# CrystalAnalyst/Lsm

Hardware: AMD Instinct MI355X
Metric: GiB/s device-resident SSTable block encode+decode, 4 KiB blocks, 1/2/4/8 GPU (higher is better)
Workload: dtype u8; 1 GPU; U: 1048576 blocks/GPU x block_size 4096, decode + re-encode (16-B uniform keys, 100-B values); blocks_per_gpu=1048576, entries_per_gpu=32474205, encoded_bytes_per_gpu=4226189427, decoded_bytes_per_gpu=4286595060, block_size=4096, segments_per_gpu=2045, parallelism=block-sharded x1 (no data-path collective), encode_output=segments packed (lsmblk_encode_batch), rccl_world=1

## Files before the change

### lsm_amd/csrc/lsmblk_dev.hpp

```cpp
#pragma once

#include <hip/hip_runtime.h>
#include <hip/hip_ext.h>

#include <cstdint>
#include <cstdlib>
#include <cstring>
#include <mutex>
#include <new>
#include <type_traits>
#include <vector>

#include "lsmblk.h"

namespace {

typedef unsigned int u32x4 __attribute__((ext_vector_type(4)));
typedef unsigned int u32x2 __attribute__((ext_vector_type(2)));
typedef __amdgpu_buffer_rsrc_t rsrc_t;

constexpr uint32_t kSpinLimit = 1u << 22;

constexpr bool kDiag = LSMBLK_DIAG_BUILD != 0;
__device__ __forceinline__ uint32_t diag_mask(uint32_t skip) { return kDiag ? skip : 0u; }

__device__ __forceinline__ uint32_t lane_id() { return threadIdx.x & 63u; }
__device__ __forceinline__ uint32_t uni(uint32_t x) { return __builtin_amdgcn_readfirstlane(x); }

__device__ __forceinline__ uint32_t xcd_tile(uint32_t b, uint32_t G) {
  const uint32_t x = b & 7, i = b >> 3, q = G >> 3, r = G & 7;
  return x * q + (x < r ? x : r) + i;
}
__device__ __forceinline__ uint64_t uni64(uint64_t x) {
  return (uint64_t(uni(uint32_t(x >> 32))) << 32) | uni(uint32_t(x));
}
__device__ __forceinline__ uint64_t lane64(uint64_t x, uint32_t j) {
  return (uint64_t(uint32_t(__builtin_amdgcn_readlane(uint32_t(x >> 32), j))) << 32) |
         uint32_t(__builtin_amdgcn_readlane(uint32_t(x), j));
}
typedef const __attribute__((address_space(4))) uint32_t cu32_t;
typedef const __attribute__((address_space(4))) uint64_t cu64_t;
__device__ __forceinline__ cu32_t* kconst(const uint32_t* p) { return (cu32_t*)p; }
__device__ __forceinline__ cu64_t* kconst(const uint64_t* p) { return (cu64_t*)p; }
__device__ __forceinline__ uint32_t wave_id() { return __builtin_amdgcn_readfirstlane(threadIdx.x >> 6); }
__device__ __forceinline__ void wave_sync() {
  __builtin_amdgcn_fence(__ATOMIC_RELEASE, "wavefront");
  __builtin_amdgcn_wave_barrier();
  __builtin_amdgcn_fence(__ATOMIC_ACQUIRE, "wavefront");
}
#define LSM_DPP(v, ctrl, rmask) uint32_t(__builtin_amdgcn_update_dpp(0u, (v), (ctrl), (rmask), 0xF, false))
__device__ __forceinline__ uint32_t wave_incl_scan32(uint32_t v) {
  v += LSM_DPP(v, 0x111, 0xF);
  v += LSM_DPP(v, 0x112, 0xF);
  v += LSM_DPP(v, 0x114, 0xF);
  v += LSM_DPP(v, 0x118, 0xF);
  v += LSM_DPP(v, 0x142, 0xA);
  v += LSM_DPP(v, 0x143, 0xC);
  return v;
}
__device__ __forceinline__ uint32_t wave_incl_max32(uint32_t v) {
  v = max(v, LSM_DPP(v, 0x111, 0xF));
  v = max(v, LSM_DPP(v, 0x112, 0xF));
  v = max(v, LSM_DPP(v, 0x114, 0xF));
  v = max(v, LSM_DPP(v, 0x118, 0xF));
  v = max(v, LSM_DPP(v, 0x142, 0xA));
  v = max(v, LSM_DPP(v, 0x143, 0xC));
  return v;
}
__device__ __forceinline__ uint32_t wave_incl_min31(uint32_t v) { return 0x7FFFFFFFu - wave_incl_max32(0x7FFFFFFFu - v); }
__device__ __forceinline__ uint32_t wave_sum32(uint32_t v) {
  return __builtin_amdgcn_readlane(wave_incl_scan32(v), 63);
}
template <typename T>
__device__ __forceinline__ T wave_incl_scan(T v) {
  if constexpr (sizeof(T) == 4) {
    return T(wave_incl_scan32(uint32_t(v)));
  } else {
    const uint32_t l = lane_id();
#pragma unroll
    for (uint32_t d = 1; d < 64; d <<= 1) {
      T t = __shfl_up(v, d, 64);
      if (l >= d) v += t;
    }
    return v;
  }
}
template <typename T>
__device__ __forceinline__ T wave_sum(T v) {
  if constexpr (sizeof(T) == 4) {
    return T(__builtin_amdgcn_readlane(wave_incl_scan32(uint32_t(v)), 63));
  } else {
#pragma unroll
    for (uint32_t d = 32; d >= 1; d >>= 1) v += __shfl_xor(v, d, 64);
    return v;
  }
}
__device__ __forceinline__ rsrc_t make_rsrc(const void* p16, uint32_t nbytes) {
  const uint32_t n = nbytes >= 0xFFFFFFF0u ? 0xFFFFFFFFu : (nbytes + 15) & ~15u;
  return __builtin_amdgcn_make_buffer_rsrc(const_cast<void*>(p16), (short)0, (int)n, 0x00020000);
}
__device__ __forceinline__ rsrc_t make_rsrc_exact(void* p16, uint32_t nbytes) {
  return __builtin_amdgcn_make_buffer_rsrc(p16, (short)0, (int)nbytes, 0x00020000);
}
__device__ __forceinline__ uint32_t bswap16(uint32_t v) { return ((v & 0xFF) << 8) | ((v >> 8) & 0xFF); }

__device__ __forceinline__ uint64_t gload(const uint64_t* p, uint32_t poll) {
  if (poll == 2)
    return __hip_atomic_fetch_or(const_cast<uint64_t*>(p), 0ull, __ATOMIC_RELAXED, __HIP_MEMORY_SCOPE_AGENT);
  return __hip_atomic_load(p, __ATOMIC_RELAXED, __HIP_MEMORY_SCOPE_AGENT);
}
__device__ __forceinline__ void gstore(uint64_t* p, uint64_t v, uint32_t poll) {
  if (poll == 2)
    (void)__hip_atomic_exchange(p, v, __ATOMIC_RELAXED, __HIP_MEMORY_SCOPE_AGENT);
  else
    __hip_atomic_store(p, v, __ATOMIC_RELAXED, __HIP_MEMORY_SCOPE_AGENT);
}

// ... 854 lines not shown
```

### lsm_amd/csrc/lsmblk_gpu.hip

```cpp
#include "lsmblk_dev.hpp"

namespace {


struct DecodeArgs {
  const uint8_t* blocks;
  const uint64_t* blk_off;
  uint64_t nblk;
  uint8_t* keys;
  uint32_t* key_off;
  uint8_t* vals;
  uint32_t* val_off;
  uint64_t* ts;
  uint64_t entry_cap, key_cap, val_cap;
  uint64_t* stats;
  const uint32_t* agg;
  const uint64_t* tile_pre;
  uint32_t tail;
  uint64_t* blk_ent;
  uint32_t skip;
  uint64_t* bagg;
  uint64_t* bbase;
  uint64_t* tagg;
  uint64_t* tinc;
  uint64_t lag;
  uint64_t lag_bytes;
  uint64_t* dbg;
  uint32_t tag, poll;
};

constexpr uint32_t kTile = 64;
constexpr uint32_t kDbgTiles = 32768, kDbgWords = 16 + 8 * kDbgTiles;
__device__ __forceinline__ void dbg_trace(uint64_t* dbg, uint64_t t, uint32_t k) {
  if (kDiag && dbg && t < kDbgTiles && lane_id() == 0) dbg[16 + 8 * t + k] = __builtin_amdgcn_s_memrealtime();
}


constexpr uint32_t kLB = 2;
constexpr uint32_t kDecMB = 2;
#ifndef LSMBLK_XEB
#define LSMBLK_XEB 4
#endif
constexpr uint32_t kEB = LSMBLK_XEB;
constexpr uint32_t kEBBlock = 2;


constexpr uint32_t kDecImg = 4128;
constexpr uint32_t kDecMaxE = 128;
constexpr uint32_t kDecKeyImg = 2176;
constexpr uint32_t kDecMapN = 256;
constexpr uint32_t kDecOut = 4032;
static_assert(kDecOut <= 16 * kDecMapN && 16 * kDecMapN <= kDecImg, "the chunk map covers the value run");

struct alignas(16) DecLds {
  uint8_t img[kDecImg];
  alignas(16) uint8_t kimg[kDecKeyImg];
  alignas(16) uint16_t cmap[kDecMapN];
};
static_assert(sizeof(DecLds) <= (160 << 10) / 24, "decode LDS: room for 24 blocks per CU");

struct DecTables {
  uint16_t epos[kDecMaxE], pfx[kDecMaxE], sfx[kDecMaxE];
  uint32_t kout[kDecMaxE + 1], vout[kDecMaxE + 1];
};
static_assert(sizeof(DecTables) <= kDecImg, "large-block tables overlay the image");

struct DecEnt {
  uint32_t epos, p, s, kout, vout, vl;
};

__device__ __forceinline__ void lds_read16(const uint8_t* base, uint32_t x, uint32_t (&v)[4]) {
  const u32x4 q = *reinterpret_cast<const u32x4*>(base + x);
  v[0] = q.x, v[1] = q.y, v[2] = q.z, v[3] = q.w;
}

constexpr int kLdAux = 0;

template <class Img>
__device__ void dec_simple_outputs(const DecodeArgs& a, const Img& im, const BlockHdr& h,
                                   uint64_t E0, uint64_t K0, uint64_t V0) {
  const uint32_t l = lane_id();
  uint64_t kc = 0, vc = 0;
  for (uint32_t c = 0; c < h.n; c += 64) {
    const uint32_t k = c + l;
    uint32_t off = 0, p = 0, s = 0, vl = 0;
    if (k < h.n) parse_entry(im, h, k, off, p, s, vl);
    const uint64_t kl = p + s;
    const uint64_t ki = wave_incl_scan<uint64_t>(kl), vi = wave_incl_scan<uint64_t>(vl);
    const uint64_t kpos = K0 + kc + ki - kl, vpos = V0 + vc + vi - vl;
    kc += __shfl(ki, 63, 64);
    vc += __shfl(vi, 63, 64);
    if (k < h.n) {
      const uint64_t e = E0 + k;
      if (e < a.entry_cap) {
        a.ts[e] = im.u64(off + 4 + s);
        a.key_off[e] = uint32_t(kpos);
        a.val_off[e] = uint32_t(vpos);
      }
      for (uint32_t t = 0; t < p; ++t)
        if (kpos + t < a.key_cap) a.keys[kpos + t] = uint8_t(im.u8(4 + t));
      for (uint32_t t = 0; t < s; ++t)
        if (kpos + p + t < a.key_cap) a.keys[kpos + p + t] = uint8_t(im.u8(off + 4 + t));
      for (uint32_t t = 0; t < vl; ++t)
        if (vpos + t < a.val_cap) a.vals[vpos + t] = uint8_t(im.u8(off + 14 + s + t));
    }
  }
}

__device__ __forceinline__ void st16(const rsrc_t& R, uint32_t off, const uint32_t (&v)[4]) {
  const u32x4 q = {v[0], v[1], v[2], v[3]};
  __builtin_amdgcn_raw_buffer_store_b128(q, R, off, 0, 0);
}

__device__ __forceinline__ void st_short(const rsrc_t& R, uint32_t off, uint32_t len, const uint32_t (&v)[4]) {
// ... 412 lines not shown
  if (total == 0) {
    after(first, 0u, ~0u);
    return;
  }
  wave_sync();
  reinterpret_cast<u32x4*>(sc)[l] = u32x4{so, dof, len - 16, first};
  uint32_t carry = 0;
  for (uint32_t g0 = 0; g0 < total; g0 += 64 * B) {
    CopyBatch<B> c;
    copy_issue<B, PIN>(RS, g0, total, np, first, sc, carry, c);
    if constexpr (PIN) copy_land(c);
    copy_store(RD, c);
    after(first, g0, g0 + 64 * B >= total ? ~0u : g0 + 64 * B);
  }
}

__device__ __forceinline__ void dec_big_entry(const DecodeArgs& a, const DecTables& L, const GlbImg& im, uint32_t k,
                                              uint32_t lim, const rsrc_t& RK, uint32_t kb, uint64_t E0, uint64_t K0,
                                              uint64_t V0) {
  const rsrc_t& R = im.r;
  const uint32_t lead = im.lead, fk = lead + 4;
  const uint32_t epos = L.epos[k], p = L.pfx[k], s = L.sfx[k], kout = L.kout[k];
  const uint32_t sb = lead + epos + 4, kl = p + s;
  const uint64_t e = E0 + k;
  a.ts[e] = im.u64(epos + 4 + s);
  a.key_off[e] = uint32_t(K0 + kout);
  a.val_off[e] = uint32_t(V0 + L.vout[k]);
  for (uint32_t t = 0; t < kl; t += 16) {
    const uint32_t o = kl >= 16 ? min(t, kl - 16) : 0u;
    uint32_t v[4];
    if (sb + o >= p && sb + o - p + 16 <= lim && fk + o + 16 <= lim) {
      const u32x4 sq = gload16(R, sb + o - p), fq = gload16(R, fk + o);
      const uint32_t sv[4] = {sq.x, sq.y, sq.z, sq.w}, fv[4] = {fq.x, fq.y, fq.z, fq.w};
#pragma unroll
      for (uint32_t d = 0; d < 4; ++d) {
        const int32_t nf = int32_t(p) - int32_t(o + 4 * d);
        const uint32_t m = nf <= 0 ? 0u : nf >= 4 ? ~0u : (1u << (8 * nf)) - 1;
        v[d] = (fv[d] & m) | (sv[d] & ~m);
      }
    } else {
#pragma unroll
      for (uint32_t d = 0; d < 4; ++d) {
        uint32_t wd = 0;
        for (uint32_t i = 0; i < 4; ++i) {
          const uint32_t x = o + 4 * d + i;
          wd |= (x < p ? im.u8(4 + x) : im.u8(epos + 4 + x - p)) << (8 * i);
        }
        v[d] = wd;
      }
    }
    if (kl >= 16) st16(RK, kb + kout + o, v);
    else st_short(RK, kb + kout, kl, v);
  }
}

#ifndef LSMBLK_XDBB
#define LSMBLK_XDBB 8
#endif
constexpr uint32_t kDecBigB = LSMBLK_XDBB;

__device__ void dec_big_outputs(const DecodeArgs& a, const DecTables& L, const rsrc_t& R, uint32_t lead,
                                const BlockHdr& h, uint32_t n, uint64_t Eb, uint64_t K0, uint64_t V0, uint32_t K,
                                uint32_t V, uint32_t* sc) {
  const uint32_t l = lane_id();
  const uint32_t kb = uint32_t(K0 & 15), vb = uint32_t(V0 & 15);
  const rsrc_t RK = make_rsrc_exact(a.keys + (K0 - kb), kb + K), RV = make_rsrc_exact(a.vals + (V0 - vb), vb + V);
  const GlbImg im{R, lead};
  const uint32_t lim = lead + h.len;
  for (uint32_t c = 0; c < n; c += 64) {
    const uint32_t k = c + l;
    const bool live = k < n;
    uint32_t vsrc = 0, vdst = 0, vl = 0;
    if (live) {
      dec_big_entry(a, L, im, k, lim, RK, kb, Eb, K0, V0);
      vsrc = lead + L.epos[k] + 14 + L.sfx[k];
      vdst = vb + L.vout[k];
      vl = L.vout[k + 1] - L.vout[k];
      if (vl < kCoop) copy_run(R, vsrc, lim, RV, vdst, vl);
    }
    copy_long_runs<kDecBigB, true>(live && vl >= kCoop, R, vsrc, RV, vdst, vl, sc);
  }
}

template <bool lagm, class Mid, class Post, class PreWait>
__device__ void decode_block(const DecodeArgs& a, DecLds& L, uint64_t b, uint64_t start, uint64_t end, Mid&& mid,
                             Post&& post, PreWait&& pre_wait) {
  const uint32_t l = lane_id();
  uint32_t err = 0;
  const uint64_t tb = b / kTile, jb = b % kTile;
  uint32_t cn = 0, ck = 0, cv = 0;
  uint64_t tp0 = 0, tp1 = 0, tp2 = 0, gb = 0;
  if constexpr (!lagm) {
    if (l < jb) {
      const uint64_t q = tb * kTile + l;
      cn = a.agg[3 * q];
      ck = a.agg[3 * q + 1];
      cv = a.agg[3 * q + 2];
    }
    tp0 = a.tile_pre[3 * tb], tp1 = a.tile_pre[3 * tb + 1], tp2 = a.tile_pre[3 * tb + 2];
  }
  uint32_t len = 0;
  if (end < start + a.tail || end - start > 0x7FFFFFF0ull) err |= LSMBLK_ERR_MALFORMED;
  else len = uint32_t(end - start) - a.tail;
  const uint8_t* bp = a.blocks + start;
  const uint32_t lead = uni(uint32_t(reinterpret_cast<uintptr_t>(bp) & 15));
  const uint8_t* abase = bp - lead;
  const rsrc_t R = make_rsrc(abase, lead + len);
  const bool fits = lead + len + 15 <= kDecImg;

  BlockHdr h;
  if (fits) {
    const uint32_t nchunk = (lead + len + 15) >> 4;
    u32x4 v[5];
    if constexpr (lagm) {
      const uint32_t o = 16 * l, o4 = o + 4096;
      asm volatile(
          "s_nop 4\n\t"
          "buffer_load_dwordx4 %0, %5, %7, 0 offen\n\t"
          "buffer_load_dwordx4 %1, %5, %7, 0 offen offset:1024\n\t"
          "buffer_load_dwordx4 %2, %5, %7, 0 offen offset:2048\n\t"
          "buffer_load_dwordx4 %3, %5, %7, 0 offen offset:3072\n\t"
          "buffer_load_dwordx4 %4, %6, %7, 0 offen"
          : "=&v"(v[0]), "=&v"(v[1]), "=&v"(v[2]), "=&v"(v[3]), "=&v"(v[4])
          : "v"(o), "v"(o4), "s"(R));
      mid();
      asm volatile("s_waitcnt vmcnt(0)" ::: "memory");
#pragma unroll
      for (uint32_t i = 0; i < 5; ++i) asm volatile("" : "+v"(v[i]));
    } else {
#pragma unroll
      for (uint32_t i = 0; i < 5; ++i)
        v[i] = __builtin_amdgcn_raw_buffer_load_b128(R, (l + 64 * i) * 16, 0, kLdAux);
    }
#pragma unroll
    for (uint32_t i = 0; i < 5; ++i)
      if (l + 64 * i < nchunk) *reinterpret_cast<u32x4*>(L.img + (l + 64 * i) * 16) = v[i];
    wave_sync();
    post();
    if (lagm && l < 3 && !(diag_mask(a.skip) & 4096)) gb = gload(a.bbase + 3 * b + l, 0);
    h = parse_hdr(LdsImg{L.img, lead}, len);
  } else {
    mid();
    post();
    if (lagm && l < 3 && !(diag_mask(a.skip) & 4096)) gb = gload(a.bbase + 3 * b + l, 0);
    h = parse_hdr(GlbImg{R, lead}, len);
  }
  if (diag_mask(a.skip) & 256) return;
  if (!h.ok) err |= LSMBLK_ERR_MALFORMED;
  const bool fast = fits && h.n <= kDecMaxE;
  const bool big = !fits;

  uint64_t K = 0, V = 0;
  bool bad = false;
  DecTables& T = *reinterpret_cast<DecTables*>(L.img);
  auto parse_tables = [&](const auto& im, uint32_t c0, uint32_t cn, uint64_t& kr, uint64_t& vr) {
    for (uint32_t c = 0; c < cn; c += 64) {
      const uint32_t k = c + l;
      uint32_t off = 0, p = 0, s = 0, vl = 0;
      bool ok = true;
      if (k < cn) ok = parse_entry(im, h, c0 + k, off, p, s, vl);
      bad = bad || !ok;
      const uint32_t kl = p + s;
      const uint32_t ki = wave_incl_scan<uint32_t>(kl), vi = wave_incl_scan<uint32_t>(vl);
      if (k < cn) {
        T.epos[k] = uint16_t(off);
        T.pfx[k] = uint16_t(p);
        T.sfx[k] = uint16_t(s);
        T.kout[k] = uint32_t(kr) + ki - kl;
        T.vout[k] = uint32_t(vr) + vi - vl;
      }
      kr += __shfl(ki, 63, 64);
      vr += __shfl(vi, 63, 64);
    }
    if (l == 0) {
      T.kout[cn] = uint32_t(kr);
      T.vout[cn] = uint32_t(vr);
    }
  };
  DecEnt ent[2] = {};
  if (fast) {
    const LdsImg im{L.img, lead};
#pragma unroll
    for (uint32_t it = 0; it < 2; ++it) {
      if (64 * it >= h.n) break;
      const uint32_t k = 64 * it + l;
      uint32_t off = 0, p = 0, s = 0, vl = 0;
      bool ok = true;
      if (k < h.n) ok = parse_entry(im, h, k, off, p, s, vl);
      bad = bad || !ok;
      const uint32_t kl = p + s;
      const uint32_t ki = wave_incl_scan<uint32_t>(kl), vi = wave_incl_scan<uint32_t>(vl);
      ent[it] = DecEnt{off, p, s, uint32_t(K) + ki - kl, uint32_t(V) + vi - vl, vl};
      K += __shfl(ki, 63, 64);
      V += __shfl(vi, 63, 64);
    }
  } else if (big && h.n <= kDecMaxE) {
    parse_tables(GlbImg{R, lead}, 0, h.n, K, V);
  } else {
    for (uint32_t c = 0; c < h.n; c += 64) {
      const uint32_t k = c + l;
      uint32_t off = 0, p = 0, s = 0, vl = 0;
      bool ok = true;
      if (k < h.n) {
        if (fits) ok = parse_entry(LdsImg{L.img, lead}, h, k, off, p, s, vl);
        else ok = parse_entry(GlbImg{R, lead}, h, k, off, p, s, vl);
      }
      bad = bad || !ok;
      K += wave_sum<uint64_t>(p + s);
      V += wave_sum<uint64_t>(vl);
    }
  }
  if (diag_mask(a.skip) & 512) return;
  if (__ballot(bad)) err |= LSMBLK_ERR_MALFORMED;
  uint64_t agg[3] = {h.n, K, V};
  if (err) agg[0] = agg[1] = agg[2] = 0;

  pre_wait();
  uint64_t excl[3];
  if constexpr (lagm) {
    const uint64_t want = (uint64_t(a.tag) << 2) | 2;
    uint32_t spins = 0;
    if (b % kTile == 0) dbg_trace(a.dbg, b / kTile, 2);
    while (!(diag_mask(a.skip) & 2048) && __ballot(l < 3 && (gb & 0xFFFF) != want)) {
      if (++spins > kSpinLimit) {
        err |= LSMBLK_ERR_TIMEOUT;
        break;
      }
      __builtin_amdgcn_s_sleep(1);
      if (l < 3 && (gb & 0xFFFF) != want) gb = gload(a.bbase + 3 * b + l, a.poll);
    }
#pragma unroll
    for (uint32_t q = 0; q < 3; ++q)
      excl[q] = uint64_t(uint32_t(__builtin_amdgcn_readlane(uint32_t(gb >> 16), q))) |
                (uint64_t(uint32_t(__builtin_amdgcn_readlane(uint32_t(gb >> 48), q))) << 32);
    if (b % kTile == 0) dbg_trace(a.dbg, b / kTile, 3);
  } else {
    excl[0] = tp0 + wave_sum(cn);
    excl[1] = tp1 + wave_sum(ck);
    excl[2] = tp2 + wave_sum(cv);
  }
  wave_sync();
  const uint64_t E0 = excl[0], K0 = excl[1], V0 = excl[2];
  if (a.blk_ent && l == 0) a.blk_ent[b] = E0;
  const uint64_t Et = E0 + agg[0], Kt = K0 + agg[1], Vt = V0 + agg[2];
  if (Kt > 0xFFFFFFFFull || Vt > 0xFFFFFFFFull) err |= LSMBLK_ERR_OVERFLOW;
  if (Et > a.entry_cap || Kt > a.key_cap || Vt > a.val_cap) err |= LSMBLK_ERR_CAPACITY;
  if (lagm && b + 1 == a.nblk && l == 0) {
    if (a.blk_ent) a.blk_ent[a.nblk] = Et;
    a.stats[0] = Et;
    a.stats[1] = Kt;
    a.stats[2] = Vt;
    if (Et <= a.entry_cap) {
      a.key_off[Et] = uint32_t(Kt);
      a.val_off[Et] = uint32_t(Vt);
    }
  }

  if (!(err & (LSMBLK_ERR_MALFORMED | LSMBLK_ERR_TIMEOUT | LSMBLK_ERR_OVERFLOW | LSMBLK_ERR_CAPACITY)) && h.n) {
    if (fast) {
      dec_fast_outputs(a, L, lead, h, ent, E0, K0, V0, uint32_t(K), uint32_t(V), diag_mask(a.skip));
    } else if (big && h.n <= kDecMaxE) {
      dec_big_outputs(a, T, R, lead, h, h.n, E0, K0, V0, uint32_t(K), uint32_t(V), reinterpret_cast<uint32_t*>(L.kimg));
    } else if (big) {
      uint64_t kr = 0, vr = 0;
      for (uint32_t c0 = 0; c0 < h.n; c0 += kDecMaxE) {
        const uint32_t nc = min(kDecMaxE, h.n - c0);
        wave_sync();
        parse_tables(GlbImg{R, lead}, c0, nc, kr, vr);
        wave_sync();
        dec_big_outputs(a, T, R, lead, h, nc, E0 + c0, K0, V0, uint32_t(K), uint32_t(V), reinterpret_cast<uint32_t*>(L.kimg));
      }
    } else if (fits) {
      dec_simple_outputs(a, LdsImg{L.img, lead}, h, E0, K0, V0);
    } else {
      dec_simple_outputs(a, GlbImg{R, lead}, h, E0, K0, V0);
    }
  }
  raise_err(a.stats, err);
}

__global__ __launch_bounds__(64) __attribute__((amdgpu_waves_per_eu(5))) void decode_kernel(DecodeArgs a) {
  __shared__ DecLds lds;
  const uint64_t b = blockIdx.x;
  decode_block<false>(a, lds, b, uni64(a.blk_off[b]), uni64(a.blk_off[b + 1]), [] {}, [] {}, [] {});
}


__device__ __forceinline__ uint64_t sat47(uint64_t v) { return v > (1ull << 47) - 1 ? (1ull << 47) - 1 : v; }

__device__ __forceinline__ void publish3(uint64_t* arr, uint64_t idx, uint64_t x0, uint64_t x1, uint64_t x2,
                                         uint32_t tag, uint32_t flag, uint32_t poll) {
  const uint32_t l = lane_id();
  const uint64_t x = l == 0 ? x0 : (l == 1 ? x1 : x2);
  if (l < 3) gstore(arr + 3 * idx + l, (sat47(x) << 16) | (uint64_t(tag) << 2) | flag, poll);
}

struct BlkCount {
  uint32_t n;
  uint64_t K, V;
  bool bad;
};
struct CntPre {
  rsrc_t R;
  uint32_t len, lead;
  bool ok, staged;
  u32x4 v[5];
};
__device__ __forceinline__ CntPre cnt_issue(const uint8_t* blocks, uint32_t tail, uint64_t start, uint64_t end) {
  const uint32_t l = lane_id();
  CntPre C;
  C.ok = !(end < start + tail || end - start > 0x7FFFFFF0ull);
  C.len = C.ok ? uint32_t(end - start) - tail : 0u;
  const uint8_t* bp = blocks + start;
  C.lead = uni(uint32_t(reinterpret_cast<uintptr_t>(bp) & 15));
  C.R = make_rsrc(bp - C.lead, C.lead + C.len);
  C.staged = C.ok && C.lead + C.len + 15 <= kDecImg;
  if (C.staged) {
#pragma unroll
    for (uint32_t i = 0; i < 5; ++i)
      C.v[i] = __builtin_amdgcn_raw_buffer_load_b128(C.R, (l + 64 * i) * 16, 0, kLdAux);
  }
  return C;
}
__device__ __forceinline__ BlkCount cnt_finish(const CntPre& C, uint8_t* img) {
  const uint32_t l = lane_id();
  BlkCount r{0, 0, 0, false};
  bool bad = false;
  auto count = [&](const auto& im) {
    const BlockHdr h = parse_hdr(im, C.len);
    if (!h.ok) {
      bad = true;
      return;
    }
    r.n = h.n;
    if constexpr (std::is_same_v<std::decay_t<decltype(im)>, GlbImg>) {
      for (uint32_t c = 0; c < h.n; c += 128) {
        const uint32_t k0 = c + l, k1 = c + 64 + l;
        const bool l0 = k0 < h.n, l1 = k1 < h.n;
        uint32_t o0, p0, s0, v0, o1, p1, s1, v1;
        const bool ok0 = parse_entry(im, h, l0 ? k0 : h.n - 1, o0, p0, s0, v0);
        const bool ok1 = parse_entry(im, h, l1 ? k1 : h.n - 1, o1, p1, s1, v1);
        if ((l0 && !ok0) || (l1 && !ok1)) bad = true;
        r.K += wave_sum<uint32_t>((l0 ? p0 + s0 : 0u) + (l1 ? p1 + s1 : 0u));
        r.V += wave_sum<uint32_t>((l0 ? v0 : 0u) + (l1 ? v1 : 0u));
      }
    } else {
      for (uint32_t c = 0; c < h.n; c += 64) {
        const uint32_t k = c + l;
        uint32_t off = 0, p = 0, s = 0, vl = 0;
        if (k < h.n && !parse_entry(im, h, k, off, p, s, vl)) bad = true;
        r.K += wave_sum<uint32_t>(p + s);
        r.V += wave_sum<uint32_t>(vl);
      }
    }
  };
  if (C.staged) {
    const uint32_t nchunk = (C.lead + C.len + 15) >> 4;
#pragma unroll
    for (uint32_t i = 0; i < 5; ++i)
      if (l + 64 * i < nchunk) *reinterpret_cast<u32x4*>(img + (l + 64 * i) * 16) = C.v[i];
    wave_sync();
    count(LdsImg{img, C.lead});
  } else if (C.ok) {
    count(GlbImg{C.R, C.lead});
  }
  if (!C.ok || __ballot(bad)) {
    r.bad = true;
    r.n = 0;
    r.K = r.V = 0;
  }
  return r;
}

struct FinPf {
  uint64_t g0, g1, g2;
};
__device__ __forceinline__ FinPf fin_prefetch(const DecodeArgs& a, uint64_t t) {
  const uint32_t l = lane_id();
  const uint64_t b0 = t * kTile, nb = min(uint64_t(kTile), a.nblk - b0);
  const uint64_t want = (uint64_t(a.tag) << 2) | 1;
  FinPf f{want, want, want};
  if (l < nb) {
    f.g0 = gload(a.bagg + 3 * (b0 + l), 0);
    f.g1 = gload(a.bagg + 3 * (b0 + l) + 1, 0);
    f.g2 = gload(a.bagg + 3 * (b0 + l) + 2, 0);
  }
  return f;
}
__device__ void lag_tile_finish(const DecodeArgs& a, uint64_t t, uint32_t& err, const FinPf* pf = nullptr) {
  const uint32_t l = lane_id();
  dbg_trace(a.dbg, t, 0);
  const uint64_t b0 = t * kTile, nb = min(uint64_t(kTile), a.nblk - b0);
  const uint64_t want = (uint64_t(a.tag) << 2) | 1;
  const bool mine = l < nb;
  const FinPf f0 = pf ? *pf : fin_prefetch(a, t);
  uint64_t g0 = f0.g0, g1 = f0.g1, g2 = f0.g2;
  uint32_t spins = 0;
  for (;;) {
    const bool here = (g0 & 0xFFFF) == want && (g1 & 0xFFFF) == want && (g2 & 0xFFFF) == want;
    if (!__ballot(!here)) break;
    if (++spins > kSpinLimit) {
      err |= LSMBLK_ERR_TIMEOUT;
      return;
    }
    __builtin_amdgcn_s_sleep(1);
    if (!here) {
      g0 = gload(a.bagg + 3 * (b0 + l), a.poll);
      g1 = gload(a.bagg + 3 * (b0 + l) + 1, a.poll);
      g2 = gload(a.bagg + 3 * (b0 + l) + 2, a.poll);
    }
  }
  const uint64_t x0 = mine ? g0 >> 16 : 0, x1 = mine ? g1 >> 16 : 0, x2 = mine ? g2 >> 16 : 0;
  const uint64_t i0 = wave_incl_scan<uint64_t>(x0), i1 = wave_incl_scan<uint64_t>(x1), i2 = wave_incl_scan<uint64_t>(x2);
  const uint64_t A[3] = {lane64(i0, 63), lane64(i1, 63), lane64(i2, 63)};
  uint64_t X[3] = {0, 0, 0};
  if (t == 0) {
    publish3(a.tinc, t, A[0], A[1], A[2], a.tag, 2, a.poll);
  } else {
    publish3(a.tagg, t, A[0], A[1], A[2], a.tag, 1, a.poll);
    const uint64_t wi = (uint64_t(a.tag) << 2) | 2;
    uint64_t g = wi;
    if (l < 3) g = gload(a.tinc + 3 * (t - 1) + l, 0);
    if (!__ballot(l < 3 && (g & 0xFFFF) != wi)) {
#pragma unroll
      for (uint32_t q = 0; q < 3; ++q)
        X[q] = uint64_t(uint32_t(__builtin_amdgcn_readlane(uint32_t(g >> 16), q))) |
               (uint64_t(uint32_t(__builtin_amdgcn_readlane(uint32_t(g >> 48), q))) << 32);
    } else {
      if (!lookback<3>(a.tagg, a.tinc, t, a.tag, a.poll, X)) {
        err |= LSMBLK_ERR_TIMEOUT;
        return;
      }
    }
    publish3(a.tinc, t, X[0] + A[0], X[1] + A[1], X[2] + A[2], a.tag, 2, a.poll);
  }
  if (mine) {
    const uint64_t tg = (uint64_t(a.tag) << 2) | 2;
    gstore(a.bbase + 3 * (b0 + l), (sat47(X[0] + i0 - x0) << 16) | tg, a.poll);
    gstore(a.bbase + 3 * (b0 + l) + 1, (sat47(X[1] + i1 - x1) << 16) | tg, a.poll);
    gstore(a.bbase + 3 * (b0 + l) + 2, (sat47(X[2] + i2 - x2) << 16) | tg, a.poll);
  }
  if (kDiag && a.dbg) {
    asm volatile("s_waitcnt vmcnt(0)" ::: "memory");
    dbg_trace(a.dbg, t, 1);
  }
}

__global__ __launch_bounds__(64) __attribute__((amdgpu_waves_per_eu(5))) void decode_lag_kernel(DecodeArgs a) {
  __shared__ DecLds lds;
  const uint32_t j = blockIdx.x, nblk = uint32_t(a.nblk), lag0 = uint32_t(a.lag);
  const bool cnt = j < nblk;
  const uint32_t l = lane_id();
  uint64_t o = 0;
  if ((l < 2 && cnt) || (l >= 2 && l < 4 && j >= lag0)) o = a.blk_off[(l < 2 ? j : j - lag0) + (l & 1)];
  const uint64_t o0 = a.lag_bytes ? a.blk_off[0] : 0, o1 = a.lag_bytes ? a.blk_off[nblk] : 0;
  const uint64_t cs = lane64(o, 0), ce = lane64(o, 1);
  CntPre C;
  const bool do_cnt = cnt && !(diag_mask(a.skip) & 1024);
  if (do_cnt) C = cnt_issue(a.blocks, a.tail, cs, ce);
  uint32_t lag = lag0;
  if (a.lag_bytes) {
    const uint32_t tot = uint32_t(min((o1 - o0) >> 12, uint64_t(0xFFFFFFFFu))), lb = uint32_t(a.lag_bytes >> 12);
    if (uint64_t(lb) * nblk < uint64_t(lag) * tot) {
      const uint32_t want = uint32_t(float(lb) * (float(nblk) / float(tot)));
      lag = want < 2 * kTile ? 2 * kTile : want;
    }
  }
  if (j >= nblk + lag) return;
  const bool dec = j >= lag;
  if (j % kTile == 0) dbg_trace(a.dbg, j / kTile, 4);
  if (dec && (j - lag) % kTile == 0) dbg_trace(a.dbg, (j - lag) / kTile, 5);
  const uint32_t b = j - lag;
  if (lag != lag0 && dec && l >= 2 && l < 4) o = a.blk_off[b + (l & 1)];
  const uint64_t ds = lane64(o, 2), de = lane64(o, 3);
  uint32_t err = 0;
  BlkCount r{0, 0, 0, false};
  auto count = [&] {
    if (!do_cnt) return;
    r = cnt_finish(C, lds.img);
    wave_sync();
  };
  const uint32_t D = lag / 2 + 63;
  const uint32_t ft = j >= D ? (j - D + 8) / kTile : ~0u;
  const bool fin = j >= D && ft * kTile + D - (ft & 7) == j && ft * kTile < nblk;
  auto publish = [&] {
    if (!cnt || (diag_mask(a.skip) & 16384)) return;
    publish3(a.bagg, j, r.n, r.K, r.V, a.tag, 1, a.poll);
    if (r.K > 0xFFFFFFFFull || r.V > 0xFFFFFFFFull) err |= LSMBLK_ERR_OVERFLOW;
  };
  FinPf fpf{};
  if (fin) fpf = fin_prefetch(a, ft);
  auto finish = [&] {
    if (fin && !(diag_mask(a.skip) & (8192 | 16384))) lag_tile_finish(a, ft, err, &fpf);
  };
  if (dec) {
    decode_block<true>(a, lds, b, ds, de, count, publish, finish);
  } else {
    count();
    publish();
    finish();
  }
  raise_err(a.stats, err);
}

struct CountArgs {
  const uint8_t* blocks;
  const uint64_t* blk_off;
  uint64_t nblk;
  uint32_t* agg;
  uint64_t* tile_sum;
  uint64_t* stats;
  uint32_t tail;
};

__global__ __launch_bounds__(64) __attribute__((amdgpu_waves_per_eu(8))) void dec_count_staged_kernel(CountArgs a) {
  __shared__ alignas(16) uint8_t img[kDecImg];
  const uint64_t b = blockIdx.x;
  const BlkCount r = cnt_finish(cnt_issue(a.blocks, a.tail, uni64(a.blk_off[b]), uni64(a.blk_off[b + 1])), img);
  uint32_t err = r.bad ? LSMBLK_ERR_MALFORMED : 0u;
  if (lane_id() == 0) {
    a.agg[3 * b] = r.n;
    a.agg[3 * b + 1] = uint32_t(r.K > 0xFFFFFFFFull ? 0xFFFFFFFFull : r.K);
    a.agg[3 * b + 2] = uint32_t(r.V > 0xFFFFFFFFull ? 0xFFFFFFFFull : r.V);
    if (r.K > 0xFFFFFFFFull || r.V > 0xFFFFFFFFull) err |= LSMBLK_ERR_OVERFLOW;
  }
  raise_err(a.stats, err);
}

struct ScanArgs {
  const uint64_t* tile_sum;
  uint64_t* tile_pre;
  uint64_t ntiles;
  uint32_t* key_off;
  uint32_t* val_off;
  uint64_t entry_cap, key_cap, val_cap;
  uint64_t* stats;
  uint64_t* blk_ent;
  uint64_t nblk;
};

__global__ __launch_bounds__(1024) void dec_scan_kernel(ScanArgs a) {
  __shared__ uint64_t wsum[16][3];
  uint64_t lo, hi;
  share1024(a.ntiles, lo, hi);
  uint64_t s[3] = {0, 0, 0}, e[3], tot[3];
#pragma unroll 8
  for (uint64_t i = lo; i < hi; ++i) {
#pragma unroll
    for (uint32_t q = 0; q < 3; ++q) s[q] += a.tile_sum[3 * i + q];
  }
  block_excl1024<3>(s, wsum, e, tot);
  for (uint64_t i = lo; i < hi; ++i) {
#pragma unroll
    for (uint32_t q = 0; q < 3; ++q) a.tile_pre[3 * i + q] = e[q];
#pragma unroll
    for (uint32_t q = 0; q < 3; ++q) e[q] += a.tile_sum[3 * i + q];
  }
  if (threadIdx.x == 0) {
    if (a.blk_ent) a.blk_ent[a.nblk] = tot[0];
    publish_totals(a.stats, tot, TotalCaps{a.entry_cap, a.key_cap, a.val_cap}, a.key_off, a.val_off, kSentIfFits);
  }
}

struct PlanArgs {
  const uint8_t* keys;
  const uint32_t* key_off;
  const uint32_t* val_off;
  uint64_t n;
  const uint32_t* seg_start;
  uint32_t nseg;
  uint32_t block_size;
  uint32_t* sz;
  uint32_t* rec_first;
  uint32_t* blk_first;
  uint64_t* blk_off;
  uint64_t blk_cap, out_cap;
  uint64_t* stats;
  uint32_t* ticket;
  uint64_t* agg;
  uint64_t* inc;
  uint32_t tag;
  uint32_t poll;
  const uint64_t* dn;
// ... 2558 lines not shown
    float t = 0.f;
    if (hipEventSynchronize(e.e1) != hipSuccess || hipEventElapsedTime(&t, e.e0, e.e1) != hipSuccess)
      return LSMBLK_E_HIP;
    uint32_t k = 0;
    while (k < *n && strncmp(out[k].name, e.name, sizeof(out[k].name) - 1) != 0) ++k;
    if (k == *n) {
      if (k == cap) return LSMBLK_E_CAPACITY;
      memset(&out[k], 0, sizeof(out[k]));
      strncpy(out[k].name, e.name, sizeof(out[k].name) - 1);
      ++*n;
    }
    out[k].launches += 1;
    out[k].ms += t;
  }
  return LSMBLK_OK;
}

int lsmblk_ctx_reserve(lsmblk_ctx* c, uint64_t max_blocks, uint64_t max_entries, uint64_t max_segments) {
  if (!c) return LSMBLK_E_INVAL;
  CallGuard call(c, nullptr);
  if (call.rc) return call.rc;
  const int rc = reserve_locked(c, max_blocks, max_entries, max_segments, nullptr);
  if (rc) return rc;
  return hipStreamSynchronize(nullptr) == hipSuccess ? LSMBLK_OK : LSMBLK_E_HIP;
}

int lsmblk_decode_batch(lsmblk_ctx* c, const uint8_t* blocks, const uint64_t* blk_off, uint64_t nblk,
                        const lsmblk_kv_stream* out, uint64_t* stats, void* stream) {
  return lsmblk_decode_batch_ex(c, blocks, blk_off, nblk, 0, 0, out, nullptr, stats, stream);
}

int lsmblk_decode_batch_ex(lsmblk_ctx* c, const uint8_t* blocks, const uint64_t* blk_off, uint64_t nblk, uint32_t tail,
                           uint32_t flags, const lsmblk_kv_stream* out, uint64_t* blk_ent, uint64_t* stats,
                           void* stream) {
  if (!c || !blk_off || !out || !stats) return LSMBLK_E_INVAL;
  if (!aligned16(out->keys) || !aligned16(out->vals) || !out->key_off || !out->val_off) return LSMBLK_E_INVAL;
  if (nblk > 0x7FFFFFFFull || tail > 16) return LSMBLK_E_INVAL;
  if ((flags & LSMBLK_DECODE_VERIFY_CRC) && tail != 4) return LSMBLK_E_INVAL;
  CallGuard call(c, stream);
  if (call.rc) return call.rc;
  hipStream_t st = call.st;
  int rc = reserve_locked(c, nblk, 0, 0, st);
  if (rc) return rc;
  if (hipMemsetAsync(stats, 0, LSMBLK_STATS_WORDS * 8, st) != hipSuccess) return LSMBLK_E_HIP;
  if (nblk == 0) {
    LSM_LAUNCH(finish_empty_decode, dim3(1), dim3(64), 0, st, out->key_off, out->val_off, out->entry_cap);
    if (blk_ent && hipMemsetAsync(blk_ent, 0, 8, st) != hipSuccess) return LSMBLK_E_HIP;
    return launch_rc();
  }
  const uint64_t ntiles = (nblk + kTile - 1) / kTile;
  const KLogRange lr(c, &c->dec_log0, &c->dec_log1);
  if (flags & LSMBLK_DECODE_VERIFY_CRC) {
    if ((rc = lsmblk_impl::ensure_crc_tabs(c, st)) || (rc = c->vcrc.grow(st, nblk + 1, 1)) || (rc = ensure_cstats(c)))
      return rc;
    if (hipMemsetAsync(c->meta_cstats, 0, LSMBLK_STATS_WORDS * 8, st) != hipSuccess) return LSMBLK_E_HIP;
    if ((rc = lsmblk_impl::launch_crc(c, blocks, blk_off, nblk, tail, c->vcrc, c->meta_cstats, st,
                                      c->dec_two_pass ? c->dec_agg.get() : nullptr)))
      return rc;
    LSM_LAUNCH(crc_verify_kernel, dim3(uint32_t((nblk + 255) / 256)), dim3(256), 0, st, blocks, blk_off, nblk,
               c->vcrc.get(), c->meta_cstats, stats);
  }
  DecodeArgs a;
  a.blocks = blocks;
  a.blk_off = blk_off;
  a.nblk = nblk;
  a.keys = out->keys;
  a.key_off = out->key_off;
  a.vals = out->vals;
  a.val_off = out->val_off;
  a.ts = out->ts;
  a.entry_cap = out->entry_cap;
  a.key_cap = out->key_cap;
  a.val_cap = out->val_cap;
  a.stats = stats;
  a.agg = c->dec_agg;
  a.tile_pre = c->tile_pre;
  a.tail = tail;
  a.blk_ent = blk_ent;
  a.skip = c->skip;
  a.bagg = a.bbase = a.tagg = a.tinc = a.dbg = nullptr;
  a.lag = a.lag_bytes = 0;
  a.tag = a.poll = 0;
  if (!c->dec_two_pass) {
    if ((rc = next_epoch(c, st))) return rc;
    a.bagg = c->lag_gran;
    a.bbase = a.bagg + 3 * c->lag_blk_cap;
    a.tagg = a.bbase + 3 * c->lag_blk_cap;
    a.tinc = a.tagg + 3 * ((c->lag_blk_cap + kTile - 1) / kTile + 1);
    a.lag = std::max<uint64_t>(2 * kTile, std::min<uint64_t>(c->dec_lag, nblk));
    a.lag_bytes = c->dec_lag_bytes;
    a.dbg = c->dbg_on ? c->dbg : nullptr;
    if (a.dbg && hipMemsetAsync(a.dbg, 0, kDbgWords * 8, st) != hipSuccess) return LSMBLK_E_HIP;
    a.tag = c->epoch;
    a.poll = c->poll;
    LSM_LAUNCH_SLOT(2, decode_lag_kernel, dim3(uint32_t(nblk + a.lag)), dim3(64), 0, st, a);
    return launch_rc();
  }
  if (!(flags & LSMBLK_DECODE_VERIFY_CRC)) {
    CountArgs ca;
    ca.blocks = blocks;
    ca.blk_off = blk_off;
    ca.nblk = nblk;
    ca.agg = c->dec_agg;
    ca.tile_sum = c->tile_sum;
    ca.stats = stats;
    ca.tail = tail;
    LSM_LAUNCH_SLOT(0, dec_count_staged_kernel, dim3(uint32_t(nblk)), dim3(64), 0, st, ca);
  }
  LSM_LAUNCH_SLOT(0, agg_tile_kernel, dim3(uint32_t((ntiles + 3) / 4)), dim3(256), 0, st, (const uint32_t*)c->dec_agg,
                  nblk, c->tile_sum.get());
  ScanArgs sa;
  sa.tile_sum = c->tile_sum;
  sa.tile_pre = c->tile_pre;
  sa.ntiles = ntiles;
  sa.key_off = out->key_off;
  sa.val_off = out->val_off;
  sa.entry_cap = out->entry_cap;
  sa.key_cap = out->key_cap;
  sa.val_cap = out->val_cap;
  sa.stats = stats;
  sa.blk_ent = blk_ent;
  sa.nblk = nblk;
  LSM_LAUNCH_SLOT(1, dec_scan_kernel, dim3(1), dim3(1024), 0, st, sa);
  LSM_LAUNCH_SLOT(2, decode_kernel, dim3(uint32_t(nblk)), dim3(64), 0, st, a);
  return launch_rc();
}

int lsmblk_encode_batch(lsmblk_ctx* c, const lsmblk_kv_stream* in, const uint32_t* seg_start, uint32_t nseg,
                        uint32_t block_size, uint8_t* out, uint64_t out_cap, uint64_t* blk_off, uint64_t blk_cap,
                        uint64_t* stats, void* stream) {
  return lsmblk_encode_batch_ex(c, in, seg_start, nseg, block_size, 0, out, out_cap, blk_off, blk_cap, nullptr, stats,
                                stream);
}

int lsmblk_encode_batch_ex(lsmblk_ctx* c, const lsmblk_kv_stream* in, const uint32_t* seg_start, uint32_t nseg,
                           uint32_t block_size, uint32_t flags, uint8_t* out, uint64_t out_cap, uint64_t* blk_off,
                           uint64_t blk_cap, uint64_t* seg_out, uint64_t* stats, void* stream) {
  if (!c || !in || !seg_start || !blk_off || !stats || !aligned16(out)) return LSMBLK_E_INVAL;
  if (in->n >= 0xFFFFFFFFull || !in->key_off || !in->val_off) return LSMBLK_E_INVAL;
  if (block_size == 0 || (flags & ~uint32_t(LSMBLK_ENCODE_SEG_SLOTS | LSMBLK_ENCODE_FRAMED))) return LSMBLK_E_INVAL;
  if ((flags & LSMBLK_ENCODE_SEG_SLOTS) && !seg_out) return LSMBLK_E_INVAL;
  CallGuard call(c, stream);
  if (call.rc) return call.rc;
  lsmblk_impl::EncodeReq q;
  q.st = call.st;
  q.in = in;
  q.seg_start = seg_start;
  q.nseg = nseg;
  q.block_size = block_size;
  q.out = out;
  q.out_cap = out_cap;
  q.blk_off = blk_off;
  q.blk_cap = blk_cap;
  q.stats = stats;
  q.flags = flags;
  q.seg_out = seg_out;
  return lsmblk_impl::encode_locked(c, q);
}

}

namespace lsmblk_impl {
int encode_locked(lsmblk_ctx* c, const EncodeReq& q) {
  hipStream_t st = q.st;
  const lsmblk_kv_stream* const in = q.in;
  const KLogRange lr(c, &c->enc_log0, &c->enc_log1);
  const bool slots = (q.flags & LSMBLK_ENCODE_SEG_SLOTS) != 0;
  const bool framed = (q.flags & LSMBLK_ENCODE_FRAMED) != 0;
  if (slots && (!q.seg_out || q.span || q.dn || q.dnseg)) return LSMBLK_E_INVAL;
  if (framed && (q.span || q.dn || q.dnseg)) return LSMBLK_E_INVAL;
  int rc = reserve_locked(c, 0, in->n, q.nseg, st);
  if (rc) return rc;
  if (hipMemsetAsync(q.stats, 0, LSMBLK_STATS_WORDS * 8, st) != hipSuccess) return LSMBLK_E_HIP;
  if (q.nseg == 0) {
    if (in->n != 0) return LSMBLK_E_INVAL;
    if (q.blk_cap >= 1 && hipMemsetAsync(q.blk_off, 0, 8, st) != hipSuccess) return LSMBLK_E_HIP;
    return LSMBLK_OK;
  }
// ... 337 lines not shown
```

Measured before the change: 1054 GiB/s.

## Move lag-decode tile finish work into dedicated finisher workgroups

```diff
diff --git a/lsm_amd/csrc/lsmblk_dev.hpp b/lsm_amd/csrc/lsmblk_dev.hpp
--- a/lsm_amd/csrc/lsmblk_dev.hpp
+++ b/lsm_amd/csrc/lsmblk_dev.hpp
@@ -33,6 +33,26 @@
 }
 __device__ __forceinline__ uint64_t uni64(uint64_t x) {
   return (uint64_t(uni(uint32_t(x >> 32))) << 32) | uni(uint32_t(x));
+}
+
+constexpr uint32_t kLagGroup = 64;
+struct LagSlot {
+  bool fin;
+  uint32_t j;
+  uint32_t t;
+};
+__host__ __device__ __forceinline__ uint32_t lag_fin_groups(uint32_t lag) { return lag / (2 * kLagGroup); }
+__host__ __device__ __forceinline__ LagSlot lag_slot(uint32_t i, uint32_t lag) {
+  const uint32_t q = i / (kLagGroup + 1), r = i % (kLagGroup + 1), dq = lag_fin_groups(lag);
+  if (r < kLagGroup) return LagSlot{false, kLagGroup * q + r, ~0u};
+  return LagSlot{true, ~0u, q >= dq ? q - dq : ~0u};
+}
+__host__ __device__ __forceinline__ uint64_t lag_worker_at(uint64_t j) { return j + j / kLagGroup; }
+__host__ __device__ __forceinline__ uint64_t lag_finisher_at(uint64_t t, uint64_t lag) {
+  return (kLagGroup + 1) * (t + lag / (2 * kLagGroup)) + kLagGroup;
+}
+__host__ __device__ __forceinline__ uint64_t lag_grid(uint64_t nblk, uint64_t lag) {
+  return lag_worker_at(nblk + lag - 1) + 1;
 }
 __device__ __forceinline__ uint64_t lane64(uint64_t x, uint32_t j) {
   return (uint64_t(uint32_t(__builtin_amdgcn_readlane(uint32_t(x >> 32), j))) << 32) |
diff --git a/lsm_amd/csrc/lsmblk_gpu.hip b/lsm_amd/csrc/lsmblk_gpu.hip
--- a/lsm_amd/csrc/lsmblk_gpu.hip
+++ b/lsm_amd/csrc/lsmblk_gpu.hip
@@ -30,6 +30,7 @@
 };
 
 constexpr uint32_t kTile = 64;
+static_assert(kTile == kLagGroup, "one finisher slot per tile of workers (lag_slot)");
 constexpr uint32_t kDbgTiles = 32768, kDbgWords = 16 + 8 * kDbgTiles;
 __device__ __forceinline__ void dbg_trace(uint64_t* dbg, uint64_t t, uint32_t k) {
   if (kDiag && dbg && t < kDbgTiles && lane_id() == 0) dbg[16 + 8 * t + k] = __builtin_amdgcn_s_memrealtime();
@@ -608,9 +609,9 @@
   }
 }
 
-template <bool lagm, class Mid, class Post, class PreWait>
+template <bool lagm, class Mid, class Post>
 __device__ void decode_block(const DecodeArgs& a, DecLds& L, uint64_t b, uint64_t start, uint64_t end, Mid&& mid,
-                             Post&& post, PreWait&& pre_wait) {
+                             Post&& post) {
   const uint32_t l = lane_id();
   uint32_t err = 0;
   const uint64_t tb = b / kTile, jb = b % kTile;
@@ -741,7 +742,6 @@
   uint64_t agg[3] = {h.n, K, V};
   if (err) agg[0] = agg[1] = agg[2] = 0;
 
-  pre_wait();
   uint64_t excl[3];
   if constexpr (lagm) {
     const uint64_t want = (uint64_t(a.tag) << 2) | 2;
@@ -808,7 +808,7 @@
 __global__ __launch_bounds__(64) __attribute__((amdgpu_waves_per_eu(5))) void decode_kernel(DecodeArgs a) {
   __shared__ DecLds lds;
   const uint64_t b = blockIdx.x;
-  decode_block<false>(a, lds, b, uni64(a.blk_off[b]), uni64(a.blk_off[b + 1]), [] {}, [] {}, [] {});
+  decode_block<false>(a, lds, b, uni64(a.blk_off[b]), uni64(a.blk_off[b + 1]), [] {}, [] {});
 }
 
 
@@ -972,9 +972,33 @@
   }
 }
 
+__device__ __forceinline__ uint32_t lag_now(const DecodeArgs& a, uint32_t nblk, uint32_t lag0, uint64_t o0, uint64_t o1) {
+  uint32_t lag = lag0;
+  if (a.lag_bytes) {
+    const uint32_t tot = uint32_t(min((o1 - o0) >> 12, uint64_t(0xFFFFFFFFu))), lb = uint32_t(a.lag_bytes >> 12);
+    if (uint64_t(lb) * nblk < uint64_t(lag) * tot) {
+      const uint32_t want = uint32_t(float(lb) * (float(nblk) / float(tot)));
+      lag = want < 2 * kTile ? 2 * kTile : min(want, lag0);
+    }
+  }
+  return lag;
+}
+
 __global__ __launch_bounds__(64) __attribute__((amdgpu_waves_per_eu(5))) void decode_lag_kernel(DecodeArgs a) {
   __shared__ DecLds lds;
-  const uint32_t j = blockIdx.x, nblk = uint32_t(a.nblk), lag0 = uint32_t(a.lag);
+  const uint32_t nblk = uint32_t(a.nblk), lag0 = uint32_t(a.lag);
+  const LagSlot slot = lag_slot(blockIdx.x, lag0);
+  if (slot.fin) {
+    const uint64_t f0 = a.lag_bytes ? a.blk_off[0] : 0, f1 = a.lag_bytes ? a.blk_off[nblk] : 0;
+    const uint32_t t = lag_slot(blockIdx.x, lag_now(a, nblk, lag0, f0, f1)).t;
+    if (t == ~0u || t * kTile >= nblk || (diag_mask(a.skip) & (8192 | 16384))) return;
+    uint32_t ferr = 0;
+    const FinPf fpf = fin_prefetch(a, t);
+    lag_tile_finish(a, t, ferr, &fpf);
+    raise_err(a.stats, ferr);
+    return;
+  }
+  const uint32_t j = slot.j;
   const bool cnt = j < nblk;
   const uint32_t l = lane_id();
   uint64_t o = 0;
@@ -984,14 +1008,7 @@
   CntPre C;
   const bool do_cnt = cnt && !(diag_mask(a.skip) & 1024);
   if (do_cnt) C = cnt_issue(a.blocks, a.tail, cs, ce);
-  uint32_t lag = lag0;
-  if (a.lag_bytes) {
-    const uint32_t tot = uint32_t(min((o1 - o0) >> 12, uint64_t(0xFFFFFFFFu))), lb = uint32_t(a.lag_bytes >> 12);
-    if (uint64_t(lb) * nblk < uint64_t(lag) * tot) {
-      const uint32_t want = uint32_t(float(lb) * (float(nblk) / float(tot)));
-      lag = want < 2 * kTile ? 2 * kTile : want;
-    }
-  }
+  const uint32_t lag = lag_now(a, nblk, lag0, o0, o1);
   if (j >= nblk + lag) return;
   const bool dec = j >= lag;
   if (j % kTile == 0) dbg_trace(a.dbg, j / kTile, 4);
@@ -1006,25 +1023,16 @@
     r = cnt_finish(C, lds.img);
     wave_sync();
   };
-  const uint32_t D = lag / 2 + 63;
-  const uint32_t ft = j >= D ? (j - D + 8) / kTile : ~0u;
-  const bool fin = j >= D && ft * kTile + D - (ft & 7) == j && ft * kTile < nblk;
   auto publish = [&] {
     if (!cnt || (diag_mask(a.skip) & 16384)) return;
     publish3(a.bagg, j, r.n, r.K, r.V, a.tag, 1, a.poll);
     if (r.K > 0xFFFFFFFFull || r.V > 0xFFFFFFFFull) err |= LSMBLK_ERR_OVERFLOW;
   };
-  FinPf fpf{};
-  if (fin) fpf = fin_prefetch(a, ft);
-  auto finish = [&] {
-    if (fin && !(diag_mask(a.skip) & (8192 | 16384))) lag_tile_finish(a, ft, err, &fpf);
-  };
   if (dec) {
-    decode_block<true>(a, lds, b, ds, de, count, publish, finish);
+    decode_block<true>(a, lds, b, ds, de, count, publish);
   } else {
     count();
     publish();
-    finish();
   }
   raise_err(a.stats, err);
 }
@@ -3749,18 +3757,20 @@
   a.lag = a.lag_bytes = 0;
   a.tag = a.poll = 0;
   if (!c->dec_two_pass) {
+    a.lag = std::max<uint64_t>(2 * kTile, std::min<uint64_t>(c->dec_lag, nblk));
+    const uint64_t grid = lag_grid(nblk, a.lag);
+    if (grid > 0x7FFFFFFFull) return LSMBLK_E_INVAL;
     if ((rc = next_epoch(c, st))) return rc;
     a.bagg = c->lag_gran;
     a.bbase = a.bagg + 3 * c->lag_blk_cap;
     a.tagg = a.bbase + 3 * c->lag_blk_cap;
     a.tinc = a.tagg + 3 * ((c->lag_blk_cap + kTile - 1) / kTile + 1);
-    a.lag = std::max<uint64_t>(2 * kTile, std::min<uint64_t>(c->dec_lag, nblk));
     a.lag_bytes = c->dec_lag_bytes;
     a.dbg = c->dbg_on ? c->dbg : nullptr;
     if (a.dbg && hipMemsetAsync(a.dbg, 0, kDbgWords * 8, st) != hipSuccess) return LSMBLK_E_HIP;
     a.tag = c->epoch;
     a.poll = c->poll;
-    LSM_LAUNCH_SLOT(2, decode_lag_kernel, dim3(uint32_t(nblk + a.lag)), dim3(64), 0, st, a);
+    LSM_LAUNCH_SLOT(2, decode_lag_kernel, dim3(uint32_t(grid)), dim3(64), 0, st, a);
     return launch_rc();
   }
   if (!(flags & LSMBLK_DECODE_VERIFY_CRC)) {
```

Measured after the change: 1059 GiB/s, median of 5. No clear change (+0.5%).
